# jiamiya/HOPE

Hardware: AMD Instinct MI355X
Metric: parallel env steps/sec (full CarParking step incl. obs + RS search) (higher is better)
Workload: dtype f64

## Files before the change

hope_amd/build.py:

```python
import os
import subprocess

_HERE = os.path.dirname(os.path.abspath(__file__))
_CSRC = os.path.join(_HERE, 'csrc')
_ROOT = os.path.dirname(_HERE)
SOURCES = ['hope_env.hip', 'hope_rs.hip', 'hope_bev.hip', 'hope_scenegen.cpp']
HEADERS = ['hope_math.h', 'hope_dev.h', 'hope_internal.h', 'hope_step_kernel.h', 'hope_obs_pair.h', 'hope_motion_pair.h', 'hope_scenegen_core.h', 'hope_scenegen_kernel.h', 'hope_curriculum_core.h', 'hope_curriculum_kernel.h', 'hope_maplevel_core.h', 'hope_maplevel_kernel.h', 'hope_planner_core.h', 'hope_planner_kernel.h', 'hope_chooser_core.h', 'hope_chooser_kernel.h', 'hope_obsnorm_core.h', 'hope_obsnorm_kernel.h', 'hope_evaltrack_core.h', 'hope_evaltrack_kernel.h', os.path.join(_ROOT, 'include', 'hope_env.h')]
FLAGS = ['--offload-arch=gfx950', '-O3', '-std=c++17', '-ffp-contract=off', '-fno-fast-math', '-fPIC', '-shared',
         '-Wno-unused-value', '-pthread']


def lib_path():
    return os.environ.get('HOPE_AMD_LIB') or os.path.join(_HERE, 'libhope_env.so')


def _stale(out):
    if not os.path.exists(out):
        return True
    t = os.path.getmtime(out)
    deps = [os.path.join(_CSRC, s) for s in SOURCES] + [h if os.path.isabs(h) else os.path.join(_CSRC, h) for h in HEADERS]
    return any(os.path.getmtime(d) > t for d in deps if os.path.exists(d))


def build_extension(force=False, verbose=False):
    out = lib_path()
    if not force and not _stale(out):
        return out
    hipcc = os.environ.get('HIPCC', '/opt/rocm/bin/hipcc')
    if not os.path.exists(hipcc):
        hipcc = 'hipcc'
    extra = os.environ.get('HOPE_BUILD_DEFS', '').split()
    cmd = [hipcc] + FLAGS + extra + ['-I' + os.path.join(_ROOT, 'include'), '-I' + _CSRC] + \
          [os.path.join(_CSRC, s) for s in SOURCES] + ['-o', out]
    if verbose:
        print(' '.join(cmd))
    subprocess.check_call(cmd)
    return out
```

hope_amd/csrc/hope_obs_pair.h:

```cpp
#pragma once
#include "hope_step_kernel.h"

namespace hope {

constexpr int OP_HALF = 32;
constexpr int OP_CAP = SMALL_TILE;
static_assert(OP_CAP == OP_HALF, "one lane per obstacle slot in the near-obstacle scan");
#ifndef HOPE_PAIR_NARROW
#define HOPE_PAIR_NARROW 6
#endif
static_assert(HOPE_PAIR_NARROW * 64 <= 512, "narrow edges of one pass must fit the pair queue");
constexpr int OP_EAGER = 16;
constexpr int OP_LQ = 512;
constexpr int OP_TILE_W = 8 * OP_CAP, OP_BEST_W = 128, OP_KLIST_W = OP_CAP / 2, OP_CFL_W = OP_CAP / 8;
constexpr int OP_HALF_W = OP_TILE_W + OP_BEST_W + OP_KLIST_W + OP_CFL_W;
constexpr size_t OP_LDS_BYTES = (size_t)2 * OP_HALF_W * 8 + (size_t)OP_LQ * 2;
static_assert(NACT == 42 && NBEAM == 120 && NBEAM <= 4 * OP_HALF, "lane layout of the pair kernel");

template <typename OT>
__global__ __launch_bounds__(64) void k_obs_pair(StepParams p) {
    extern __shared__ __attribute__((aligned(16))) double lds[];
    const int lane = threadIdx.x, hw = lane >> 5, hl = lane & (OP_HALF - 1);
    const int n_pairs = (p.n_list + 1) >> 1;
    if ((int)blockIdx.x >= n_pairs) return;
    const int li = 2 * scene_of_block(blockIdx.x, n_pairs) + hw;
    bool live = li < p.n_list;
    const int scene = p.scene_list[live ? li : li - 1];
    if (p.active) live = live && p.active[scene] != 0;
    if (!__any(live)) return;

    double* hbase = lds + hw * OP_HALF_W;
    double* tile = hbase;
    unsigned long long* best = (unsigned long long*)(hbase + OP_TILE_W);
    int* klist = (int*)(hbase + OP_TILE_W + OP_BEST_W);
    uint8_t* cfl = (uint8_t*)(klist + OP_CAP);
    uint16_t* queue = (uint16_t*)(lds + 2 * OP_HALF_W);

    const int n_obst = live ? min(p.n_obst[scene], OP_CAP) : 0;
    const double* st = p.state + (size_t)scene * ST_WORDS;
    const double x = st[0], y = st[1];
    const double ct = p.cs[2 * (size_t)scene], sn = p.cs[2 * (size_t)scene + 1];
    const float4* obb_s = p.obb + (size_t)scene * p.max_obst;
    float4 bb = make_float4(0.0f, 0.0f, 0.0f, 0.0f);
    if (hl < OP_EAGER) bb = obb_s[hl];
    const uint8_t gfl = (p.eflag + (size_t)scene * eflag_stride(p.max_obst))[hl];
    const double2* src = (const double2*)(p.verts + (size_t)scene * p.max_obst * 8);

    if (hl >= OP_EAGER && hl < n_obst) bb = obb_s[hl];
    const double lr = LIDAR_RANGE + 1e-6;
    const bool near = hl < n_obst && !((double)bb.x > x + lr || (double)bb.y < x - lr || (double)bb.z > y + lr || (double)bb.w < y - lr);
    int n_l;
    {
        const unsigned long long m = __ballot(near);
        const unsigned hm = hw ? (unsigned)(m >> 32) : (unsigned)m;
        n_l = __popc(hm);
        if (near) {
            const int pos = __popc(hm & ((1u << hl) - 1));
            klist[pos] = hl;
            cfl[pos] = gfl;
        }
    }
    ssync();
    for (int i = hl; i < 4 * n_l; i += OP_HALF) ((double2*)tile)[i] = src[4 * klist[i >> 2] + (i & 3)];
    double base[4], pm[4];
#pragma unroll
    for (int r = 0; r < 4; r++) {
        const int bi = hl + OP_HALF * r;
        base[r] = bi < NBEAM ? p.hull_base[bi] : 0.0;
        pm[r] = bi < NBEAM ? (HOPE_MASK_LUT ? p.mask_bsc[bi] : p.pmax[UPS * bi]) : 0.0;
    }
#pragma unroll
    for (int r = 0; r < 4; r++) best[hl + OP_HALF * r] = 0x7ff0000000000000ull;
    ssync();
    {
        const double a = ct, b = sn;
        const double x_off = -x * a - y * b;
        const double y_off = x * b - y * a;
        for (int i = hl; i < 4 * n_l; i += OP_HALF) {
            const double px = tile[2 * i], py = tile[2 * i + 1];
            tile[2 * i] = a * px + b * py + x_off;
            tile[2 * i + 1] = (-b) * px + a * py + y_off;
        }
    }
    ssync();
    const int nl_max = max(__builtin_amdgcn_readlane(n_l, 0), __builtin_amdgcn_readlane(n_l, OP_HALF));
    int n_k = 0;
    for (int base_i = 0; base_i < 4 * nl_max; base_i += OP_HALF) {
        const int i = base_i + hl;
        const bool in = i < 4 * n_l;
        const int o = in ? i >> 2 : 0;
        double dd = INFINITY;
        bool amb;
        {
            bool keep_c = false, drop_c = false;
            if (in) {
                const int e = 4 * o + (i & 3), e2 = 4 * o + ((i + 1) & 3);
                const double ax = tile[2 * e], ay = tile[2 * e + 1], bx = tile[2 * e2], by = tile[2 * e2 + 1];
                const double ddx = bx - ax, ddy = by - ay;
                const double len2 = ddx * ddx + ddy * ddy;
                const double dot = (0.0 - ax) * ddx + (0.0 - ay) * ddy;
                const double qa = ax * ax + ay * ay, qb = bx * bx + by * by;
                const double num = ay * ddx - ax * ddy;
                const double R2 = LIDAR_RANGE * LIDAR_RANGE, ETA = 1e-9;
                const double lo = R2 * (1.0 - ETA), hi = R2 * (1.0 + ETA);
                const double n2 = num * num;
                const bool line_far = n2 > hi * len2, line_near = n2 < lo * len2;
                const bool foot_in = dot > ETA * len2 && dot < (1.0 - ETA) * len2;
                const bool foot_a = dot < -ETA * len2, foot_b = dot > (1.0 + ETA) * len2;
                keep_c = qa < lo || qb < lo || (foot_in && line_near);
                drop_c = !keep_c && (len2 > 0.0 ? (line_far || (foot_a && qa > hi) || (foot_b && qb > hi)) : qa > hi);
            }
            const unsigned long long kb = __ballot(keep_c), db = __ballot(drop_c);
            const int sh = lane & ~3;
            const bool ring_keep = ((kb >> sh) & 0xF) != 0, ring_drop = ((db >> sh) & 0xF) == 0xF;
            if (ring_keep) dd = 0.0;
            amb = in && !ring_keep && !ring_drop;
        }
        if (__any(amb)) {
            if (amb) {
                const int e = 4 * o + (i & 3), e2 = 4 * o + ((i + 1) & 3);
                dd = origin_seg_dist(tile[2 * e], tile[2 * e + 1], tile[2 * e2], tile[2 * e2 + 1]);
            }
            dd = fmin(dd, dpp_d<0xB1>(dd));
            dd = fmin(dd, dpp_d<0x4E>(dd));
        }
        const bool kq = in && (i & 3) == 0 && dd < LIDAR_RANGE;
        const unsigned long long km = __ballot(kq);
        const unsigned hkm = hw ? (unsigned)(km >> 32) : (unsigned)km;
        if (kq) klist[n_k + __popc(hkm & ((1u << hl) - 1))] = o;
        n_k += __popc(hkm);
    }
    ssync();
    const int n_kslots = 4 * n_k;
    const int nk_max = max(__builtin_amdgcn_readlane(n_kslots, 0), __builtin_amdgcn_readlane(n_kslots, OP_HALF));

    int qn = 0;
    auto drain = [&]() {
        ssync();
        for (int q0 = 0; q0 < qn; q0 += WAVE) {
            const int q = q0 + lane;
            if (q < qn) {
                const int pr = queue[q];
                const int bi = pr & 127, e = (pr >> 7) & 127, hh = pr >> 14;
                const int e2 = (e & ~3) | ((e + 1) & 3);
                const double* tl = lds + hh * OP_HALF_W;
                const double x1 = tl[2 * e], y1 = tl[2 * e + 1], x2 = tl[2 * e2], y2 = tl[2 * e2 + 1];
                const double d = y2 - y1, ee = x1 - x2, f = y1 * x2 - x1 * y2;
                const double ba = p.beam_ab[2 * bi], bb_ = p.beam_ab[2 * bi + 1];
                double r = INFINITY;
                if (beam_may_hit(ba, bb_, x1, y1, x2, y2)) r = beam_edge(bi, ba, bb_, x1, y1, x2, y2, d, ee, f);
                if (r < INFINITY) atomicMin((unsigned long long*)(tl + OP_TILE_W) + bi, (unsigned long long)__double_as_longlong(r));
            }
        }
        ssync();
        qn = 0;
    };
    {
        const float PITCH = 6.283185307179586f / NBEAM, MARGIN = 2e-3f;
        for (int base_i = 0; base_i < nk_max && !(p.stages & STAGE_NO_BEAMS); base_i += OP_HALF) {
            const int i = base_i + hl;
            const bool in = i < n_kslots;
            const int e = in ? 4 * klist[i >> 2] + (i & 3) : 0;
            int lo = 0, cnt = 0;
            bool front = false, back = false, risky = true;
            if (in) {
                const int e2 = (e & ~3) | ((e + 1) & 3);
                const double dx1 = tile[2 * e], dy1 = tile[2 * e + 1], dx2 = tile[2 * e2], dy2 = tile[2 * e2 + 1];
                const float x1 = (float)dx1, y1 = (float)dy1;
                const float x2 = (float)dx2, y2 = (float)dy2;
                const float t1 = span_angle(y1, x1);
                const float t2 = __int_as_float(__builtin_amdgcn_mov_dpp(__float_as_int(t1), 0x39, 0xf, 0xf, true));
                float dth = t2 - t1;
                if (dth > 3.14159265f) dth -= 6.28318531f;
                if (dth <= -3.14159265f) dth += 6.28318531f;
                const float span = fabsf(dth);
                const bool wild = span > 3.13f || !(span == span) || fminf(x1 * x1 + y1 * y1, x2 * x2 + y2 * y2) < 0.01f;
                if (wild) { lo = 0; cnt = NBEAM; }
                else {
                    float ts = dth >= 0 ? t1 : t2;
                    if (ts < 0) ts += 6.28318531f;
                    const int ilo = (int)ceilf((ts - MARGIN) * (1.0f / PITCH));
                    const int ihi = (int)floorf((ts + span + MARGIN) * (1.0f / PITCH));
                    cnt = ihi - ilo + 1;
                    if (cnt < 0) cnt = 0;
                    if (cnt > NBEAM) cnt = NBEAM;
                    lo = ilo < 0 ? ilo + NBEAM : ilo >= NBEAM ? ilo - NBEAM : ilo;
                    if ((unsigned)lo >= (unsigned)NBEAM) { lo = 0; cnt = NBEAM; }
                }
                const int fl = (int)cfl[e >> 2];
                const double cr = dx1 * dy2 - dx2 * dy1;
                const double sc2 = (dx1 * dx1 + dy1 * dy1) * (dx2 * dx2 + dy2 * dy2);
                const bool decisive = cr * cr > 1e-12 * sc2;
                const bool left = cr > 0;
                front = decisive && (left != ((fl & OBST_F_CCW) != 0));
                back = decisive && !front;
                const float q1 = t1 * (1.0f / PITCH);
                const bool near_beam = fabsf(q1 - rintf(q1)) * PITCH <= 2.0e-4f + 1e-5f;
                const bool thin = front && (fabs(dx2 - dx1) < 1e-4 || fabs(dy2 - dy1) < 1e-4);
                risky = wild || !decisive || near_beam || thin || !(fl & OBST_F_CONVEX);
            }
            {
                const unsigned long long rb = __ballot(risky), fb = __ballot(front), bb2 = __ballot(back);
                const int sh = lane & ~3;
                const bool ring_ok = ((rb >> sh) & 0xF) == 0 && ((fb >> sh) & 0xF) != 0 && ((bb2 >> sh) & 0xF) != 0;
                if (ring_ok && back && !(p.stages & STAGE_NO_CULL)) cnt = 0;
            }
            constexpr int NARROW = HOPE_PAIR_NARROW;
            const int tag = (hw << 14) | (e << 7);
            const int cs = (cnt > 0 && cnt <= NARROW) ? cnt : 0;
            const int incl = wave_incl_scan_i(cs, lane);
            const int total = __builtin_amdgcn_readlane(incl, WAVE - 1);
            if (total > 0) {
                if (qn + total > OP_LQ) drain();
                const int off = qn + incl - cs;
#pragma unroll
                for (int k = 0; k < NARROW; k++) {
                    if (k < cs) {
                        int bi = lo + k;
                        if (bi >= NBEAM) bi -= NBEAM;
                        queue[off + k] = (uint16_t)(tag | bi);
                    }
                }
                qn += total;
            }
            unsigned long long todo = __ballot(cnt > NARROW);
            while (todo) {
                const int el = __ffsll((long long)todo) - 1;
                todo &= todo - 1;
                const int lo_e = __builtin_amdgcn_readlane(lo, el), cnt_e = __builtin_amdgcn_readlane(cnt, el);
                if (qn + cnt_e > OP_LQ) drain();
                const int tag_e = __builtin_amdgcn_readlane(tag, el);
                if (lane < cnt_e) {
                    int bi = lo_e + lane;
                    if (bi >= NBEAM) bi -= NBEAM;
                    queue[qn + lane] = (uint16_t)(tag_e | bi);
                }
                if (cnt_e > WAVE && lane + WAVE < cnt_e) {
                    int bi = lo_e + lane + WAVE;
                    if (bi >= NBEAM) bi -= NBEAM;
                    queue[qn + lane + WAVE] = (uint16_t)(tag_e | bi);
                }
                qn += cnt_e;
            }
        }
    }
    if (qn > 0) drain();
    else ssync();

    double lid[4];
#pragma unroll
    for (int r = 0; r < 4; r++) {
        const int bi = hl + OP_HALF * r;
        const double bq = sqrt(__longlong_as_double((long long)best[bi < NBEAM ? bi : 0]));
        lid[r] = clipd(bq, 0, LIDAR_RANGE) - base[r];
    }
    if (p.lidar && live) {
        OT* lo_ = (OT*)p.lidar + (size_t)NBEAM * scene;
#pragma unroll
        for (int r = 0; r < 4; r++) {
            const int bi = hl + OP_HALF * r;
            if (bi < NBEAM) lo_[bi] = (OT)lid[r];
        }
    }
    if (!p.action_mask || (p.stages & STAGE_NO_MASK)) return;

    ssync();
    double* xs = (double*)best;
    double xv_own[4];
#pragma unroll
    for (int r = 0; r < 4; r++) {
        const int bi = hl + OP_HALF * r;
        xv_own[r] = clipd(lid[r], 0, 10) + base[r];
        if (bi < NBEAM) xs[bi] = xv_own[r];
    }
    if (hl == 0) xs[NBEAM] = xv_own[0];
    constexpr int HALF_ACT = NACT / 2;
    const bool alane = hl < HALF_ACT;
    int ms[2] = {NITER, NITER};
    bool tie = false;
#if HOPE_MASK_LUT
    uint32_t* alist = (uint32_t*)tile;
    int n_act = 0;
#pragma unroll
    for (int r = 0; r < 4; r++) {
        const int bi = hl + OP_HALF * r;
        const double q = (xv_own[r] - (base[r] - 1e-6)) * pm[r];
        const bool c = live && bi < NBEAM && q < (double)MASK_LUT_NB;
        const unsigned long long m = __ballot(c);
        const unsigned hm = hw ? (unsigned)(m >> 32) : (unsigned)m;
        if (c) alist[n_act + __popc(hm & ((1u << hl) - 1))] = (uint32_t)(bi << 16) | (uint32_t)(bi * MASK_LUT_NB + (int)q);
        n_act += __popc(hm);
    }
    ssync();
    const int na_max = max(__builtin_amdgcn_readlane(n_act, 0), __builtin_amdgcn_readlane(n_act, OP_HALF));
    if (na_max > 0) {
        constexpr uint32_t NONE = (uint32_t)(NBEAM * MASK_LUT_NB);
        const char* lutb = (const char*)p.mask_lut + 2 * hl;
        unsigned mlo[2] = {NITER, NITER}, mhi[2] = {NITER, NITER};
        constexpr int PG = 8;
        unsigned pk[PG / 2];
        {
            unsigned v0[PG];
#pragma unroll
            for (int g = 0; g < PG; g++) {
                const uint32_t e = g < n_act ? alist[g] & 0xFFFFu : NONE;
                v0[g] = *(const uint16_t*)(lutb + e * (MASK_LUT_ROW * 2u));
            }
#pragma unroll
            for (int g = 0; g < PG; g++) {
                mlo[0] = min(mlo[0], v0[g] & 15u); mhi[0] = min(mhi[0], (v0[g] >> 4) & 15u);
                mlo[1] = min(mlo[1], (v0[g] >> 8) & 15u); mhi[1] = min(mhi[1], v0[g] >> 12);
            }
#pragma unroll
            for (int g = 0; g < PG / 2; g++) pk[g] = v0[2 * g] | v0[2 * g + 1] << 16;
        }
        for (int k0 = PG; k0 < na_max; k0 += PG) {
            unsigned v[PG];
#pragma unroll
            for (int g = 0; g < PG; g++) {
                const uint32_t e = k0 + g < n_act ? alist[k0 + g] & 0xFFFFu : NONE;
                v[g] = *(const uint16_t*)(lutb + e * (MASK_LUT_ROW * 2u));
            }
#pragma unroll
            for (int g = 0; g < PG; g++) {
                mlo[0] = min(mlo[0], v[g] & 15u); mhi[0] = min(mhi[0], (v[g] >> 4) & 15u);
                mlo[1] = min(mlo[1], (v[g] >> 8) & 15u); mhi[1] = min(mhi[1], v[g] >> 12);
            }
        }
        if (__any(mlo[0] < mhi[0] || mlo[1] < mhi[1])) {
// ... 181 lines not shown
```

hope_amd/csrc/hope_step_kernel.h:

```cpp
#pragma once
#include "hope_dev.h"
#ifndef HOPE_PART0_OCC
#define HOPE_PART0_OCC 4
#endif
#ifndef HOPE_KIN_PRIO
#define HOPE_KIN_PRIO 3
#endif
#ifndef HOPE_MASK_MG
#define HOPE_MASK_MG 4
#endif
#include "hope_env.h"
#include "hope_internal.h"
#ifndef HOPE_STEP_SYNC_FULL
#define HOPE_STEP_SYNC_FULL 0
#endif
#ifndef HOPE_MASK_LUT
#define HOPE_MASK_LUT 1
#endif
#ifndef HOPE_MASK_FRAC_TABLE
#define HOPE_MASK_FRAC_TABLE 0
#endif

namespace hope {

// ... 389 lines not shown
    }
    return false;
}

constexpr float SPAN_ANGLE_C[6] = {0.9999772310256958f, -0.33262282609939575f, 0.19354036450386047f,
                                   -0.11642643809318542f, 0.05264730006456375f, -0.01171911507844925f};
__device__ __forceinline__ float span_angle(float y, float x) {
    const float ax = fabsf(x), ay = fabsf(y);
    const float mx = fmaxf(ax, ay), mn = fminf(ax, ay);
    const float t = mn * __builtin_amdgcn_rcpf(mx);
    const float s = t * t;
    float q = __builtin_fmaf(s, SPAN_ANGLE_C[5], SPAN_ANGLE_C[4]);
    q = __builtin_fmaf(q, s, SPAN_ANGLE_C[3]);
    q = __builtin_fmaf(q, s, SPAN_ANGLE_C[2]);
    q = __builtin_fmaf(q, s, SPAN_ANGLE_C[1]);
    q = __builtin_fmaf(q, s, SPAN_ANGLE_C[0]);
    float r = q * t;
    if (ay > ax) r = 1.57079633f - r;
    if (x < 0.0f) r = 3.14159265f - r;
    return copysignf(r, y);
}

__device__ __forceinline__ double origin_seg_dist(double ax, double ay, double bx, double by) {
    if (ax == bx && ay == by) return sqrt(ax * ax + ay * ay);
    double len2 = (bx - ax) * (bx - ax) + (by - ay) * (by - ay);
    double r = ((0.0 - ax) * (bx - ax) + (0.0 - ay) * (by - ay)) / len2;
    if (r <= 0.0) return sqrt(ax * ax + ay * ay);
    if (r >= 1.0) return sqrt(bx * bx + by * by);
    double s = ((ay - 0.0) * (bx - ax) - (ax - 0.0) * (by - ay)) / len2;
    return fabs(s) * sqrt(len2);
}

__device__ __forceinline__ bool beam_may_hit(double a, double b, double x1, double y1, double x2, double y2) {
    double s1 = a * x1 + b * y1, s2 = a * x2 + b * y2;
    const double eps = 1e-9, back = -1e-6;
    if ((s1 > eps && s2 > eps) || (s1 < -eps && s2 < -eps)) return false;
    double t1 = a * y1 - b * x1, t2 = a * y2 - b * x2;
    if (t1 < back && t2 < back) return false;
    return true;
}

__device__ __forceinline__ double beam_edge(int i, double a, double b, double x1, double y1, double x2, double y2,
                                            double d, double e, double f) {
    double det = a * e - b * d;
    if (det == 0) return INFINITY;
    double raw_x = (b * f) / det;
    double raw_y = (-(a * f)) / det;
    const double tz = 1e-8;
    const double sx = (i < NBEAM / 4 || i >= NBEAM / 4 * 3) ? 1.0 : -1.0, sy = (i < NBEAM / 2) ? 1.0 : -1.0;
    bool ok = !(sx * raw_x < -tz) && !(sy * raw_y < -tz);
    ok = ok && !(raw_x > fmax(x1, x2)) && !(raw_x < fmin(x1, x2));
    ok = ok && !(raw_y > fmax(y1, y2)) && !(raw_y < fmin(y1, y2));
    return ok ? raw_x * raw_x + raw_y * raw_y : INFINITY;
}

constexpr int KIN_SCENES_PER_BLOCK = WAVE / 4;

__constant__ const double MASK_STEP_FRACTION[NITER + 1] = {0.0 / NITER, 1.0 / NITER, 2.0 / NITER, 3.0 / NITER, 4.0 / NITER, 5.0 / NITER,
                                                           6.0 / NITER, 7.0 / NITER, 8.0 / NITER, 9.0 / NITER, 10.0 / NITER};
static_assert(NITER == 10, "MASK_STEP_FRACTION lists NITER + 1 quotients");

__device__ __forceinline__ int wave_incl_scan_i(int x, int lane) {
    x += __builtin_amdgcn_update_dpp(0, x, 0x111, 0xf, 0xf, false);
    x += __builtin_amdgcn_update_dpp(0, x, 0x112, 0xf, 0xf, false);
    x += __builtin_amdgcn_update_dpp(0, x, 0x114, 0xf, 0xf, false);
    x += __builtin_amdgcn_update_dpp(0, x, 0x118, 0xf, 0xf, false);
    const int t0 = __builtin_amdgcn_readlane(x, 15), t1 = __builtin_amdgcn_readlane(x, 31), t2 = __builtin_amdgcn_readlane(x, 47);
    return x + (lane >= 16 ? t0 : 0) + (lane >= 32 ? t1 : 0) + (lane >= 48 ? t2 : 0);
}

template <int CTRL>
__device__ __forceinline__ double dpp_d(double v) {
    const int hi = __builtin_amdgcn_mov_dpp(__double2hiint(v), CTRL, 0xf, 0xf, true);
    const int lo = __builtin_amdgcn_mov_dpp(__double2loint(v), CTRL, 0xf, 0xf, true);
    return __hiloint2double(hi, lo);
}

template <int J>
__device__ __forceinline__ double quad_bcast(double v) {
    const int hi = __builtin_amdgcn_mov_dpp(__double2hiint(v), J * 0x55, 0xf, 0xf, true);
    const int lo = __builtin_amdgcn_mov_dpp(__double2loint(v), J * 0x55, 0xf, 0xf, true);
    return __hiloint2double(hi, lo);
}

static_assert(MINI_ITER == 20, "div_by_20");
__device__ __forceinline__ double div_by_20(double x) {
    const double R = 0.05;
    const double q0 = x * R;
    const double r = fma(-q0, 20.0, x);
    return copysign(fma(r, R, q0), x);
}

template <typename AT>
__device__ __forceinline__ void kin_controls(const void* actions, int scene, uint32_t stages, double& speed, double& dh) {
    const AT* act = (const AT*)actions;
    const double a0 = (double)act[2 * (size_t)scene], a1 = (double)act[2 * (size_t)scene + 1];
    double steer = a0;
    speed = a1;
    if (!(stages & HOPE_ACTION_PHYSICAL)) {
        if (sizeof(AT) == 4 && (stages & HOPE_ACTION_RESCALE_F32)) {
            const float f0 = fminf(fmaxf((float)a0, -1.0f), 1.0f), f1 = fminf(fmaxf((float)a1, -1.0f), 1.0f);
            steer = (double)(f0 * ((float)STEER_HI - (float)STEER_LO) / 2.0f + ((float)STEER_HI + (float)STEER_LO) / 2.0f);
            speed = (double)(f1 * ((float)SPEED_HI - (float)SPEED_LO) / 2.0f + ((float)SPEED_HI + (float)SPEED_LO) / 2.0f);
        } else {
            steer = clipd(a0, -1, 1) * (STEER_HI - STEER_LO) / 2 + (STEER_HI + STEER_LO) / 2;
            speed = clipd(a1, -1, 1) * (SPEED_HI - SPEED_LO) / 2 + (SPEED_HI + SPEED_LO) / 2;
        }
    }
    speed = clipd(speed, SPEED_LO, SPEED_HI);
    steer = clipd(steer, STEER_LO, STEER_HI);
    dh = speed * hm_tan(steer) / WHEEL_BASE * STEP_LENGTH / MINI_ITER;
}

template <typename AT>
__global__ __launch_bounds__(64) void k_kinematics(int n, const int32_t* scene_list, const double* state, const void* actions,
                                                  const uint8_t* active, uint32_t stages, const double* scene_c, double* kin) {
    if (HOPE_KIN_PRIO) __builtin_amdgcn_s_setprio(HOPE_KIN_PRIO);
    __shared__ double buf[KIN_SCENES_PER_BLOCK * KIN_WORDS];
    __shared__ double terms[MINI_ITER][2 * KIN_SCENES_PER_BLOCK];
    __shared__ int sid[KIN_SCENES_PER_BLOCK];
#ifdef HOPE_KIN_PAD
    __shared__ double kin_pad[HOPE_KIN_PAD];
    if (n < 0) kin_pad[threadIdx.x] = 0.0, kin[0] = kin_pad[(threadIdx.x * 7) % HOPE_KIN_PAD];
#endif
    const int lane = threadIdx.x, q = lane & 3, ls = lane >> 2;
    const int idx = blockIdx.x * KIN_SCENES_PER_BLOCK + ls;
    const int scene = idx < n ? (scene_list ? scene_list[idx] : idx) : -1;
    const bool live = scene >= 0 && !(active && !active[scene]);
    if (__all(!live)) return;
    if (q == 0) sid[ls] = live ? scene : -1;
    const int sc_ = live ? scene : 0;
    const double* st = state + (size_t)sc_ * ST_WORDS;
    double h = st[2];
    double acc = 0.0;
    if (lane < 2 * KIN_SCENES_PER_BLOCK) {
        const int idx2 = blockIdx.x * KIN_SCENES_PER_BLOCK + (lane >> 1);
        const int sc2 = idx2 < n ? (scene_list ? scene_list[idx2] : idx2) : 0;
        acc = state[(size_t)sc2 * ST_WORDS + (lane & 1)];
    }
    double speed, dh;
    kin_controls<AT>(actions, sc_, stages, speed, dh);
    double* out = buf + ls * KIN_WORDS;
    for (int i = 0; i < q; i++) h = h + dh;
    constexpr int KJ = MINI_ITER / 4;
    static_assert(MINI_ITER % 4 == 0, "micro-steps per lane and round");
#pragma unroll 1
    for (int r = 0; r < NUM_STEP; r++) {
        double hj[KJ], sj[KJ], cj[KJ];
        hj[0] = h;
#pragma unroll
        for (int j = 1; j < KJ; j++) { double t = hj[j - 1]; t = t + dh; t = t + dh; t = t + dh; t = t + dh; hj[j] = t; }
#pragma unroll
        for (int j = 0; j < KJ; j++) hm_sincos(hj[j], &sj[j], &cj[j]);
        if (q == 0 && r > 0) {
            const int k = r - 1;
            out[k] = hj[0]; out[10 + k] = cj[0]; out[20 + k] = sj[0];
        }
#pragma unroll
        for (int j = 0; j < KJ; j++) {
            terms[4 * j + q][2 * ls] = div_by_20(speed * cj[j] * STEP_LENGTH);
            terms[4 * j + q][2 * ls + 1] = div_by_20(speed * sj[j] * STEP_LENGTH);
        }
        ssync();
        if (lane < 2 * KIN_SCENES_PER_BLOCK) {
#pragma unroll
            for (int m = 0; m < MINI_ITER; m++) acc += terms[m][lane];
// ... 436 lines not shown
            pr[0] = prev_x; pr[1] = prev_y; pr[2] = prev_h; pr[3] = fin_x; pr[4] = fin_y; pr[5] = fin_h; pr[6] = fin_ua;
            const int fl = ((p.stages & HOPE_STAGE_REWARD) ? POST_F_REWARD : 0) | (turnover ? POST_F_TURNOVER : 0) | (need_ua ? POST_F_NEED_UA : 0);
            pr[7] = __hiloint2double(fl, status | (fin_t << 8));
        }
    }

    }
    if (PART == 1 || !(p.stages & HOPE_STAGE_OBS)) { ST_T(2); ST_FLUSH(); return; }

    ST_T(2);
    int* llist = keep;
    ssync();
    const double lr = LIDAR_RANGE + 1e-6;
    const uint8_t* eflag_s = p.eflag + (size_t)scene * eflag_stride(p.max_obst);
    const int n_l = PART == 2 ? stage_near(obb_s, src, n_obst, x - lr, x + lr, y - lr, y + lr, tile, llist, lane, eflag_s, cfl, &obb_pre)
                              : build_near_list(tile, n_obst, x, y, lr, llist, lane);
    ssync();
    {
        const double a = ct, b = sn;
        const double x_off = -x * a - y * b;
        const double y_off = x * b - y * a;
        for (int i = lane; i < 4 * n_l; i += WAVE) {
            const int v = 4 * llist[i >> 2] + (i & 3);
            double px = tile[2 * v], py = tile[2 * v + 1];
            tile[2 * v] = a * px + b * py + x_off;
            tile[2 * v + 1] = (-b) * px + a * py + y_off;
        }
    }
    ssync();
    int n_k = 0;
    for (int base = 0; base < 4 * n_l; base += WAVE) {
        const int i = base + lane;
        const bool in = i < 4 * n_l;
        const int o = in ? llist[i >> 2] : 0;
        double dd = INFINITY;
        bool amb = in;
        if (!TIMING) {
            bool keep_c = false, drop_c = false;
            if (in) {
                const int e = 4 * o + (i & 3), e2 = 4 * o + ((i + 1) & 3);
                const double ax = tile[2 * e], ay = tile[2 * e + 1], bx = tile[2 * e2], by = tile[2 * e2 + 1];
                const double ddx = bx - ax, ddy = by - ay;
                const double len2 = ddx * ddx + ddy * ddy;
                const double dot = (0.0 - ax) * ddx + (0.0 - ay) * ddy;
                const double qa = ax * ax + ay * ay, qb = bx * bx + by * by;
                const double num = ay * ddx - ax * ddy;
                const double R2 = LIDAR_RANGE * LIDAR_RANGE, ETA = 1e-9;
                const double lo = R2 * (1.0 - ETA), hi = R2 * (1.0 + ETA);
                const double n2 = num * num;
                const bool line_far = n2 > hi * len2, line_near = n2 < lo * len2;
                const bool foot_in = dot > ETA * len2 && dot < (1.0 - ETA) * len2;
                const bool foot_a = dot < -ETA * len2, foot_b = dot > (1.0 + ETA) * len2;
                keep_c = qa < lo || qb < lo || (foot_in && line_near);
                drop_c = !keep_c && (len2 > 0.0 ? (line_far || (foot_a && qa > hi) || (foot_b && qb > hi)) : qa > hi);
            }
            const unsigned long long kb = __ballot(keep_c), db = __ballot(drop_c);
            const int sh = lane & ~3;
            const bool ring_keep = ((kb >> sh) & 0xF) != 0, ring_drop = ((db >> sh) & 0xF) == 0xF;
            if (ring_keep) dd = 0.0;
            amb = in && !ring_keep && !ring_drop;
        }
        if (__any(amb)) {
            if (amb) {
                const int e = 4 * o + (i & 3), e2 = 4 * o + ((i + 1) & 3);
                dd = origin_seg_dist(tile[2 * e], tile[2 * e + 1], tile[2 * e2], tile[2 * e2 + 1]);
            }
            dd = fmin(dd, dpp_d<0xB1>(dd));
            dd = fmin(dd, dpp_d<0x4E>(dd));
        }
        if (TIMING && in && (i & 3) == 0) { cen_ring_n += 1; cen_ring = fmin(cen_ring, fabs(dd - LIDAR_RANGE)); }
        const bool kq = in && (i & 3) == 0 && dd < LIDAR_RANGE;
        const unsigned long long km = __ballot(kq);
        if (kq) llist[n_k + __popcll(km & ((1ull << lane) - 1))] = o;
        n_k += __popcll(km);
    }
    ssync();
    const int n_kslots = 4 * n_k;
    ST_T(3);
    const int i0 = lane, i1 = lane + 64;
    const bool has1 = i1 < NBEAM;
    const double a0 = PART == 2 ? bm0 : p.beam_ab[2 * i0], b0 = PART == 2 ? bm1 : p.beam_ab[2 * i0 + 1];
    const double a1 = PART == 2 ? bm2 : (has1 ? p.beam_ab[2 * i1] : 0.0), b1 = PART == 2 ? bm3 : (has1 ? p.beam_ab[2 * i1 + 1] : 0.0);
    unsigned long long* best = (unsigned long long*)(scr + LDS_TX);
    int* queue = (int*)(scr + LDS_TX + 128);
    constexpr int LQ = 384;
    best[lane] = 0x7ff0000000000000ull;
    best[lane + 64] = 0x7ff0000000000000ull;
    ssync();
    int qn = 0;
    auto drain = [&]() {
        const unsigned long long td_ = TIMING ? __builtin_readcyclecounter() : 0;
        ssync();
        for (int q0 = 0; q0 < qn; q0 += WAVE) {
            int q = q0 + lane;
            if (q < qn) {
                int pr = queue[q];
                int bi = pr & 127, e = pr >> 7;
                int e2 = (e & ~3) | ((e + 1) & 3);
                double x1 = tile[2 * e], y1 = tile[2 * e + 1], x2 = tile[2 * e2], y2 = tile[2 * e2 + 1];
                double d = y2 - y1, ee = x1 - x2, f = y1 * x2 - x1 * y2;
                const double ba = p.beam_ab[2 * bi], bb = p.beam_ab[2 * bi + 1];
                double r = INFINITY;
                if (beam_may_hit(ba, bb, x1, y1, x2, y2)) r = beam_edge(bi, ba, bb, x1, y1, x2, y2, d, ee, f);
                if (r < INFINITY) atomicMin(&best[bi], (unsigned long long)__double_as_longlong(r));
            }
        }
        ssync();
        qn = 0;
        if (TIMING) { const unsigned long long dt_ = __builtin_readcyclecounter() - td_; tsec[6] += dt_; t0_ += dt_; }
    };
    {
        const float PITCH = 6.283185307179586f / NBEAM, MARGIN = 2e-3f;
        for (int base = 0; base < n_kslots && !(p.stages & STAGE_NO_BEAMS); base += WAVE) {
            const int i = base + lane;
            const int e = i < n_kslots ? 4 * llist[i >> 2] + (i & 3) : 0;
            int lo = 0, cnt = 0;
            bool front = false, back = false, risky = true;
            if (i < n_kslots) {
                const int e2 = (e & ~3) | ((e + 1) & 3);
                const double dx1 = tile[2 * e], dy1 = tile[2 * e + 1], dx2 = tile[2 * e2], dy2 = tile[2 * e2 + 1];
                const float x1 = (float)dx1, y1 = (float)dy1;
                const float x2 = (float)dx2, y2 = (float)dy2;
                const float t1 = span_angle(y1, x1);
                const float t2 = __int_as_float(__builtin_amdgcn_mov_dpp(__float_as_int(t1), 0x39, 0xf, 0xf, true));
                float dth = t2 - t1;
                if (dth > 3.14159265f) dth -= 6.28318531f;
                if (dth <= -3.14159265f) dth += 6.28318531f;
                const float span = fabsf(dth);
                const bool wild = span > 3.13f || !(span == span) || fminf(x1 * x1 + y1 * y1, x2 * x2 + y2 * y2) < 0.01f;
                if (wild) { lo = 0; cnt = NBEAM; }
                else {
                    float ts = dth >= 0 ? t1 : t2;
                    if (ts < 0) ts += 6.28318531f;
                    const int ilo = (int)ceilf((ts - MARGIN) * (1.0f / PITCH));
                    const int ihi = (int)floorf((ts + span + MARGIN) * (1.0f / PITCH));
                    cnt = ihi - ilo + 1;
                    if (cnt < 0) cnt = 0;
                    if (cnt > NBEAM) cnt = NBEAM;
                    lo = ilo < 0 ? ilo + NBEAM : ilo >= NBEAM ? ilo - NBEAM : ilo;
                    if ((unsigned)lo >= (unsigned)NBEAM) { lo = 0; cnt = NBEAM; }
                }
                const int fl = (int)cfl[e >> 2];
                const double cr = dx1 * dy2 - dx2 * dy1;
                const double sc2 = (dx1 * dx1 + dy1 * dy1) * (dx2 * dx2 + dy2 * dy2);
                const bool decisive = cr * cr > 1e-12 * sc2;
                const bool left = cr > 0;
                front = decisive && (left != ((fl & OBST_F_CCW) != 0));
                back = decisive && !front;
                const float q1 = t1 * (1.0f / PITCH);
                const bool near_beam = fabsf(q1 - rintf(q1)) * PITCH <= 2.0e-4f + 1e-5f;
                const bool thin = front && (fabs(dx2 - dx1) < 1e-4 || fabs(dy2 - dy1) < 1e-4);
                risky = wild || !decisive || near_beam || thin || !(fl & OBST_F_CONVEX);
            }
            {
                const unsigned long long rb = __ballot(risky), fb = __ballot(front), bb = __ballot(back);
                const int sh = lane & ~3;
                const bool ring_ok = ((rb >> sh) & 0xF) == 0 && ((fb >> sh) & 0xF) != 0 && ((bb >> sh) & 0xF) != 0;
                if (ring_ok && back && !(p.stages & STAGE_NO_CULL)) cnt = 0;
            }
            ST_T(4);
            constexpr int NARROW = 6;
            const int cs = (cnt > 0 && cnt <= NARROW) ? cnt : 0;
            const int incl = wave_incl_scan_i(cs, lane);
            const int total = __builtin_amdgcn_readlane(incl, WAVE - 1);
            if (total > 0) {
                if (qn + total > LQ) drain();
                const int off = qn + incl - cs, tag = e << 7;
#pragma unroll
                for (int k = 0; k < NARROW; k++) {
                    if (k < cs) {
                        int bi = lo + k;
                        if (bi >= NBEAM) bi -= NBEAM;
                        queue[off + k] = tag | bi;
                    }
                }
                qn += total;
            }
            unsigned long long todo = __ballot(cnt > NARROW);
            while (todo) {
                const int el = __ffsll((long long)todo) - 1;
                todo &= todo - 1;
                const int lo_e = __builtin_amdgcn_readlane(lo, el), cnt_e = __builtin_amdgcn_readlane(cnt, el);
                if (qn + cnt_e > LQ) drain();
                const int tag = __builtin_amdgcn_readlane(e, el) << 7;
                if (lane < cnt_e) {
                    int bi = lo_e + lane;
                    if (bi >= NBEAM) bi -= NBEAM;
                    queue[qn + lane] = tag | bi;
                }
                if (cnt_e > WAVE && lane + WAVE < cnt_e) {
                    int bi = lo_e + lane + WAVE;
                    if (bi >= NBEAM) bi -= NBEAM;
                    queue[qn + lane + WAVE] = tag | bi;
                }
                qn += cnt_e;
            }
            ST_T(5);
        }
    }
    constexpr bool MLUT = HOPE_MASK_LUT && !TIMING;
    const double pm0 = MLUT ? p.mask_bsc[i0] : p.pmax[UPS * i0], pm1 = has1 ? (MLUT ? p.mask_bsc[i1] : p.pmax[UPS * i1]) : 0.0;
    if (qn > 0) drain();
    const double best0 = sqrt(__longlong_as_double((long long)best[i0]));
    const double best1 = has1 ? sqrt(__longlong_as_double((long long)best[i1])) : INFINITY;
    const double base0 = p.hull_base[i0], base1 = has1 ? p.hull_base[i1] : 0.0;
    const double lid0 = clipd(best0, 0, LIDAR_RANGE) - base0;
    const double lid1 = clipd(best1, 0, LIDAR_RANGE) - base1;
    if (p.lidar) {
        OT* lo = (OT*)p.lidar + (size_t)NBEAM * scene;
        lo[i0] = (OT)lid0;
        if (has1) lo[i1] = (OT)lid1;
    }
    ST_T(5);
    if (!p.action_mask || (p.stages & STAGE_NO_MASK)) { ST_FLUSH(); return; }

    ssync();
    double* xs = scr + LDS_X;
    xs[i0] = clipd(lid0, 0, 10) + base0;
    if (has1) xs[i1] = clipd(lid1, 0, 10) + base1;
    ssync();
    if (lane == 0) xs[NBEAM] = xs[0];
    ssync();
    int mstep = NITER;
    bool tie = false, mask_trivial = false;
    if (MLUT) {
        const double q0 = (xs[i0] - (base0 - 1e-6)) * pm0, q1 = has1 ? (xs[i1] - (base1 - 1e-6)) * pm1 : (double)MASK_LUT_NB;
        const bool c0 = q0 < (double)MASK_LUT_NB, c1 = has1 && q1 < (double)MASK_LUT_NB;
        const int row0 = i0 * MASK_LUT_NB + (c0 ? (int)q0 : 0), row1 = i1 * MASK_LUT_NB + (c1 ? (int)q1 : 0);
        const unsigned long long am[2] = {__ballot(c0), __ballot(c1)};
        mask_trivial = !(am[0] | am[1]);
        if (am[0] | am[1]) {
            constexpr int NONE = NBEAM * MASK_LUT_NB;
            const int hl_ = lane < NACT / 2 ? lane : (lane < NACT ? lane - NACT / 2 : 31), sh_ = (lane >= NACT / 2 && lane < NACT) ? 8 : 0;
            const char* lutb = (const char*)p.mask_lut + 2 * hl_;
            unsigned mlo = NITER, mhi = NITER;
            constexpr int PG = 8;
            unsigned long long m0 = am[0], m1 = am[1];
            auto pop_row = [&]() -> int {
                int row = NONE;
                if (m0) { const int l_ = __ffsll((long long)m0) - 1; m0 &= m0 - 1; row = __builtin_amdgcn_readlane(row0, l_); }
                else if (m1) { const int l_ = __ffsll((long long)m1) - 1; m1 &= m1 - 1; row = __builtin_amdgcn_readlane(row1, l_); }
                return row;
            };
            unsigned pk[PG / 2];
            {
                unsigned v0[PG];
#pragma unroll
                for (int g = 0; g < PG; g++) v0[g] = (unsigned)*(const uint16_t*)(lutb + (unsigned)pop_row() * (MASK_LUT_ROW * 2u)) >> sh_ & 0xFFu;
#pragma unroll
                for (int g = 0; g < PG; g++) { mlo = min(mlo, v0[g] & 15u); mhi = min(mhi, v0[g] >> 4); }
#pragma unroll
                for (int g = 0; g < PG / 2; g++) pk[g] = v0[2 * g] | v0[2 * g + 1] << 16;
            }
            while (m0 | m1) {
                unsigned v[PG];
#pragma unroll
                for (int g = 0; g < PG; g++) v[g] = (unsigned)*(const uint16_t*)(lutb + (unsigned)pop_row() * (MASK_LUT_ROW * 2u)) >> sh_ & 0xFFu;
#pragma unroll
                for (int g = 0; g < PG; g++) { mlo = min(mlo, v[g] & 15u); mhi = min(mhi, v[g] >> 4); }
            }
            if (__any(mlo < mhi)) {
                const char* tabb = (const char*)p.tab;
                int k = 0;
#pragma unroll
                for (int half = 0; half < 2; half++) {
                    unsigned long long m = am[half];
                    while (m) {
                        const int l_ = __ffsll((long long)m) - 1;
                        m &= m - 1;
                        const int ib = 64 * half + l_;
                        unsigned w;
                        switch (k >> 1) {
                            case 0: w = pk[0]; break; case 1: w = pk[1]; break; case 2: w = pk[2]; break; case 3: w = pk[3]; break;
                            default: {
                                const int row = __builtin_amdgcn_readlane(half ? row1 : row0, l_);
                                w = ((unsigned)*(const uint16_t*)(lutb + (unsigned)row * (MASK_LUT_ROW * 2u)) >> sh_ & 0xFFu) << ((k & 1) << 4);
                            }
                        }
                        w = (w >> ((k & 1) << 4)) & 0xFFu;
                        k++;
                        const unsigned lo = w & 15u, hi = w >> 4;
                        const bool need = lo < hi && lo < mhi;
                        if (!__any(need)) continue;
                        const double xv = xs[ib];
                        if (need) {
// ... 247 lines not shown
```

Baseline: 158.5 million.

## Replace per-pair lidar queue with run-length queue and skip hit prefilter for non-wild edges

Replaces the per-(edge,beam) pair queue in the lidar stage with a run-length queue. Each edge now appends one packed run descriptor plus a start mark, instead of one queue entry per beam. Drain expands runs with a wave max-scan over the marks. The two-path narrow/wide enqueue with serialized per-edge readlane loops is removed, and the beam_may_hit prefilter is skipped for non-wild edges whose beam range is already tight. This cuts enqueue work and LDS writes, at the cost of a DPP scan per drain chunk, and relies on the angular range being exact enough to drop the prefilter.

```diff
diff --git a/hope_amd/build.py b/hope_amd/build.py
--- a/hope_amd/build.py
+++ b/hope_amd/build.py
@@ -5,7 +5,7 @@
 _CSRC = os.path.join(_HERE, 'csrc')
 _ROOT = os.path.dirname(_HERE)
 SOURCES = ['hope_env.hip', 'hope_rs.hip', 'hope_bev.hip', 'hope_scenegen.cpp']
-HEADERS = ['hope_math.h', 'hope_dev.h', 'hope_internal.h', 'hope_step_kernel.h', 'hope_obs_pair.h', 'hope_motion_pair.h', 'hope_scenegen_core.h', 'hope_scenegen_kernel.h', 'hope_curriculum_core.h', 'hope_curriculum_kernel.h', 'hope_maplevel_core.h', 'hope_maplevel_kernel.h', 'hope_planner_core.h', 'hope_planner_kernel.h', 'hope_chooser_core.h', 'hope_chooser_kernel.h', 'hope_obsnorm_core.h', 'hope_obsnorm_kernel.h', 'hope_evaltrack_core.h', 'hope_evaltrack_kernel.h', os.path.join(_ROOT, 'include', 'hope_env.h')]
+HEADERS = ['hope_math.h', 'hope_dev.h', 'hope_internal.h', 'hope_step_kernel.h', 'hope_lidar_runs_core.h', 'hope_lidar_runs.h', 'hope_obs_pair.h', 'hope_motion_pair.h', 'hope_scenegen_core.h', 'hope_scenegen_kernel.h', 'hope_curriculum_core.h', 'hope_curriculum_kernel.h', 'hope_maplevel_core.h', 'hope_maplevel_kernel.h', 'hope_planner_core.h', 'hope_planner_kernel.h', 'hope_chooser_core.h', 'hope_chooser_kernel.h', 'hope_obsnorm_core.h', 'hope_obsnorm_kernel.h', 'hope_evaltrack_core.h', 'hope_evaltrack_kernel.h', os.path.join(_ROOT, 'include', 'hope_env.h')]
 FLAGS = ['--offload-arch=gfx950', '-O3', '-std=c++17', '-ffp-contract=off', '-fno-fast-math', '-fPIC', '-shared',
          '-Wno-unused-value', '-pthread']
 
diff --git a/hope_amd/csrc/hope_lidar_runs.h b/hope_amd/csrc/hope_lidar_runs.h
--- /dev/null
+++ b/hope_amd/csrc/hope_lidar_runs.h
@@ -0,0 +1,93 @@
+#pragma once
+#include "hope_lidar_runs_core.h"
+
+namespace hope {
+
+static_assert(LR_NBEAM == NBEAM && LR_WAVE == WAVE, "hope_lidar_runs_core.h restates the beam count and the wave size");
+constexpr size_t LR_LDS_BYTES = (size_t)LR_RUNS * 4 + LR_CAP;
+
+struct LidarRuns {
+    uint32_t* info;
+    uint8_t* mark;
+    int qslots, nruns;
+};
+
+__device__ __forceinline__ void lr_init(LidarRuns& Q, void* mem, int lane) {
+    Q.info = (uint32_t*)mem;
+    Q.mark = (uint8_t*)(Q.info + LR_RUNS);
+    Q.qslots = 0;
+    Q.nruns = 0;
+    static_assert(LR_CAP / 4 == 2 * WAVE, "two words of marks per lane");
+    ((uint32_t*)Q.mark)[lane] = 0;
+    ((uint32_t*)Q.mark)[lane + WAVE] = 0;
+}
+
+__device__ __forceinline__ int wave_incl_max_i(int x) {
+    x = lr_join(x, __builtin_amdgcn_update_dpp(0, x, 0x111, 0xf, 0xf, false));
+    x = lr_join(x, __builtin_amdgcn_update_dpp(0, x, 0x112, 0xf, 0xf, false));
+    x = lr_join(x, __builtin_amdgcn_update_dpp(0, x, 0x114, 0xf, 0xf, false));
+    x = lr_join(x, __builtin_amdgcn_update_dpp(0, x, 0x118, 0xf, 0xf, false));
+    x = lr_join(x, __builtin_amdgcn_update_dpp(0, x, 0x142, 0xa, 0xf, false));
+    x = lr_join(x, __builtin_amdgcn_update_dpp(0, x, 0x143, 0xc, 0xf, false));
+    return x;
+}
+
+template <class PairFn>
+__device__ __forceinline__ void lr_drain(LidarRuns& Q, int lane, PairFn pair) {
+    ssync();
+    int carry = 0;
+    for (int q0 = 0; q0 < Q.qslots; q0 += WAVE) {
+        const int q = q0 + lane;
+        int m = Q.mark[q];
+        Q.mark[q] = 0;
+        m = lr_join(wave_incl_max_i(m), carry);
+        carry = __builtin_amdgcn_readlane(m, WAVE - 1);
+        if (q < Q.qslots) {
+            const uint32_t in = Q.info[m - 1];
+            pair(in, lr_beam(in, q));
+        }
+    }
+    ssync();
+    Q.qslots = 0;
+    Q.nruns = 0;
+}
+
+template <class DrainFn>
+__device__ __forceinline__ void lr_append(LidarRuns& Q, int lane, int half, int e, int lo, int cnt, bool wild, DrainFn drain) {
+    const int incl = wave_incl_scan_i(cnt, lane);
+    const bool has = cnt > 0;
+    const unsigned long long hm = __ballot(has);
+    if (hm == 0) return;
+    const int rank = __popcll(hm & ((1ull << lane) - 1));
+    unsigned long long pend = hm;
+    int done_s = 0, done_r = 0;
+    while (pend) {
+        const bool fit = ((pend >> lane) & 1) && lr_fits(Q.qslots + (incl - done_s), Q.nruns + (rank - done_r));
+        const unsigned long long fm = __ballot(fit);
+        if (fm == 0) { drain(); continue; }
+        if (fit) {
+            const int run = Q.nruns + rank - done_r, first = Q.qslots + incl - cnt - done_s;
+            Q.info[run] = lr_pack(half, e, lo, first, wild);
+            Q.mark[first] = (uint8_t)(run + 1);
+        }
+        const int end_s = __builtin_amdgcn_readlane(incl, 63 - __clzll((long long)fm));
+        const int n = __popcll(fm);
+        Q.qslots += end_s - done_s;
+        done_s = end_s;
+        Q.nruns += n;
+        done_r += n;
+        pend &= ~fm;
+    }
+}
+
+__device__ __forceinline__ void lidar_pair(const double* tile, unsigned long long* best, const double* beam_ab, int e, int bi, bool wild) {
+    const int e2 = (e & ~3) | ((e + 1) & 3);
+    const double x1 = tile[2 * e], y1 = tile[2 * e + 1], x2 = tile[2 * e2], y2 = tile[2 * e2 + 1];
+    const double d = y2 - y1, ee = x1 - x2, f = y1 * x2 - x1 * y2;
+    const double ba = beam_ab[2 * bi], bb = beam_ab[2 * bi + 1];
+    double r = INFINITY;
+    if (!wild || beam_may_hit(ba, bb, x1, y1, x2, y2)) r = beam_edge(bi, ba, bb, x1, y1, x2, y2, d, ee, f);
+    if (r < INFINITY) atomicMin(best + bi, (unsigned long long)__double_as_longlong(r));
+}
+
+}
diff --git a/hope_amd/csrc/hope_lidar_runs_core.h b/hope_amd/csrc/hope_lidar_runs_core.h
--- /dev/null
+++ b/hope_amd/csrc/hope_lidar_runs_core.h
@@ -0,0 +1,100 @@
+#pragma once
+#include <stdint.h>
+
+#if defined(__HIPCC__) || defined(__CUDACC__)
+#define LR_HD __host__ __device__ inline
+#else
+#define LR_HD inline
+#endif
+
+constexpr int LR_NBEAM = 120;
+constexpr int LR_WAVE = 64;
+constexpr int LR_CAP = 512;
+constexpr int LR_RUNS = 128;
+static_assert(LR_CAP % LR_WAVE == 0 && LR_NBEAM <= LR_CAP && LR_RUNS < 256 && LR_CAP <= 512, "run queue layout");
+
+LR_HD uint32_t lr_pack(int half, int edge, int lo, int first, bool wild) {
+    return (uint32_t)first | (uint32_t)lo << 9 | (uint32_t)edge << 16 | (uint32_t)half << 26 | (uint32_t)(wild ? 1 : 0) << 27;
+}
+LR_HD int lr_first(uint32_t info) { return (int)(info & 511u); }
+LR_HD int lr_lo(uint32_t info) { return (int)((info >> 9) & 127u); }
+LR_HD int lr_edge(uint32_t info) { return (int)((info >> 16) & 1023u); }
+LR_HD int lr_half(uint32_t info) { return (int)((info >> 26) & 1u); }
+LR_HD bool lr_wild(uint32_t info) { return ((info >> 27) & 1u) != 0; }
+
+LR_HD int lr_beam(uint32_t info, int slot) {
+    const int b = lr_lo(info) + (slot - lr_first(info));
+    return b >= LR_NBEAM ? b - LR_NBEAM : b;
+}
+
+LR_HD bool lr_fits(int slots_after, int run) { return slots_after <= LR_CAP && run < LR_RUNS; }
+
+LR_HD int lr_join(int a, int b) { return a > b ? a : b; }
+
+#if !defined(__HIP_DEVICE_COMPILE__)
+struct LrHostQueue {
+    uint8_t mark[LR_CAP];
+    uint32_t info[LR_RUNS];
+    int qslots, nruns;
+    long drains;
+};
+inline void lr_host_init(LrHostQueue* q) {
+    for (int i = 0; i < LR_CAP; i++) q->mark[i] = 0;
+    q->qslots = q->nruns = 0;
+    q->drains = 0;
+}
+template <class Emit>
+inline void lr_host_drain(LrHostQueue* q, Emit emit) {
+    int carry = 0;
+    for (int q0 = 0; q0 < q->qslots; q0 += LR_WAVE) {
+        int m[LR_WAVE];
+        for (int lane = 0; lane < LR_WAVE; lane++) {
+            m[lane] = q->mark[q0 + lane];
+            q->mark[q0 + lane] = 0;
+        }
+        for (int lane = 1; lane < LR_WAVE; lane++) m[lane] = lr_join(m[lane], m[lane - 1]);
+        for (int lane = 0; lane < LR_WAVE; lane++) m[lane] = lr_join(m[lane], carry);
+        carry = m[LR_WAVE - 1];
+        for (int lane = 0; lane < LR_WAVE; lane++) {
+            const int s = q0 + lane;
+            if (s >= q->qslots) continue;
+            const uint32_t in = q->info[m[lane] - 1];
+            emit(lr_half(in), lr_edge(in), lr_beam(in, s), lr_wild(in));
+        }
+    }
+    q->qslots = q->nruns = 0;
+    q->drains++;
+}
+template <class Emit>
+inline void lr_host_append(LrHostQueue* q, int n, const int* half, const int* edge, const int* lo, const int* cnt, const int* wild, Emit emit) {
+    int incl[LR_WAVE], rank[LR_WAVE];
+    bool pend[LR_WAVE];
+    int s = 0, r = 0, n_pend = 0;
+    for (int k = 0; k < n; k++) {
+        rank[k] = r;
+        s += cnt[k];
+        incl[k] = s;
+        pend[k] = cnt[k] > 0;
+        if (pend[k]) { r++; n_pend++; }
+    }
+    int done_s = 0, done_r = 0;
+    while (n_pend > 0) {
+        int n_fit = 0, last = -1;
+        for (int k = 0; k < n; k++) {
+            if (!pend[k] || !lr_fits(q->qslots + (incl[k] - done_s), q->nruns + (rank[k] - done_r))) continue;
+            const int run = q->nruns + rank[k] - done_r, first = q->qslots + incl[k] - cnt[k] - done_s;
+            q->info[run] = lr_pack(half[k], edge[k], lo[k], first, wild[k] != 0);
+            q->mark[first] = (uint8_t)(run + 1);
+            pend[k] = false;
+            n_fit++;
+            last = k;
+        }
+        if (n_fit == 0) { lr_host_drain(q, emit); continue; }
+        q->qslots += incl[last] - done_s;
+        done_s = incl[last];
+        q->nruns += n_fit;
+        done_r += n_fit;
+        n_pend -= n_fit;
+    }
+}
+#endif
diff --git a/hope_amd/csrc/hope_obs_pair.h b/hope_amd/csrc/hope_obs_pair.h
--- a/hope_amd/csrc/hope_obs_pair.h
+++ b/hope_amd/csrc/hope_obs_pair.h
@@ -6,15 +6,10 @@
 constexpr int OP_HALF = 32;
 constexpr int OP_CAP = SMALL_TILE;
 static_assert(OP_CAP == OP_HALF, "one lane per obstacle slot in the near-obstacle scan");
-#ifndef HOPE_PAIR_NARROW
-#define HOPE_PAIR_NARROW 6
-#endif
-static_assert(HOPE_PAIR_NARROW * 64 <= 512, "narrow edges of one pass must fit the pair queue");
 constexpr int OP_EAGER = 16;
-constexpr int OP_LQ = 512;
 constexpr int OP_TILE_W = 8 * OP_CAP, OP_BEST_W = 128, OP_KLIST_W = OP_CAP / 2, OP_CFL_W = OP_CAP / 8;
 constexpr int OP_HALF_W = OP_TILE_W + OP_BEST_W + OP_KLIST_W + OP_CFL_W;
-constexpr size_t OP_LDS_BYTES = (size_t)2 * OP_HALF_W * 8 + (size_t)OP_LQ * 2;
+constexpr size_t OP_LDS_BYTES = (size_t)2 * OP_HALF_W * 8 + LR_LDS_BYTES;
 static_assert(NACT == 42 && NBEAM == 120 && NBEAM <= 4 * OP_HALF, "lane layout of the pair kernel");
 
 template <typename OT>
@@ -134,26 +129,13 @@
     const int n_kslots = 4 * n_k;
     const int nk_max = max(__builtin_amdgcn_readlane(n_kslots, 0), __builtin_amdgcn_readlane(n_kslots, OP_HALF));
 
-    int qn = 0;
+    LidarRuns rq;
+    lr_init(rq, lds + 2 * OP_HALF_W, lane);
     auto drain = [&]() {
-        ssync();
-        for (int q0 = 0; q0 < qn; q0 += WAVE) {
-            const int q = q0 + lane;
-            if (q < qn) {
-                const int pr = queue[q];
-                const int bi = pr & 127, e = (pr >> 7) & 127, hh = pr >> 14;
-                const int e2 = (e & ~3) | ((e + 1) & 3);
-                const double* tl = lds + hh * OP_HALF_W;
-                const double x1 = tl[2 * e], y1 = tl[2 * e + 1], x2 = tl[2 * e2], y2 = tl[2 * e2 + 1];
-                const double d = y2 - y1, ee = x1 - x2, f = y1 * x2 - x1 * y2;
-                const double ba = p.beam_ab[2 * bi], bb_ = p.beam_ab[2 * bi + 1];
-                double r = INFINITY;
-                if (beam_may_hit(ba, bb_, x1, y1, x2, y2)) r = beam_edge(bi, ba, bb_, x1, y1, x2, y2, d, ee, f);
-                if (r < INFINITY) atomicMin((unsigned long long*)(tl + OP_TILE_W) + bi, (unsigned long long)__double_as_longlong(r));
-            }
-        }
-        ssync();
-        qn = 0;
+        lr_drain(rq, lane, [&](uint32_t in, int bi) {
+            const double* tl = lds + lr_half(in) * OP_HALF_W;
+            lidar_pair(tl, (unsigned long long*)(tl + OP_TILE_W), p.beam_ab, lr_edge(in), bi, lr_wild(in));
+        });
     };
     {
         const float PITCH = 6.283185307179586f / NBEAM, MARGIN = 2e-3f;
@@ -162,7 +144,7 @@
             const bool in = i < n_kslots;
             const int e = in ? 4 * klist[i >> 2] + (i & 3) : 0;
             int lo = 0, cnt = 0;
-            bool front = false, back = false, risky = true;
+            bool front = false, back = false, risky = true, wild_e = false;
             if (in) {
                 const int e2 = (e & ~3) | ((e + 1) & 3);
                 const double dx1 = tile[2 * e], dy1 = tile[2 * e + 1], dx2 = tile[2 * e2], dy2 = tile[2 * e2 + 1];
@@ -175,6 +157,7 @@
                 if (dth <= -3.14159265f) dth += 6.28318531f;
                 const float span = fabsf(dth);
                 const bool wild = span > 3.13f || !(span == span) || fminf(x1 * x1 + y1 * y1, x2 * x2 + y2 * y2) < 0.01f;
+                wild_e = wild;
                 if (wild) { lo = 0; cnt = NBEAM; }
                 else {
                     float ts = dth >= 0 ? t1 : t2;
@@ -205,46 +188,10 @@
                 const bool ring_ok = ((rb >> sh) & 0xF) == 0 && ((fb >> sh) & 0xF) != 0 && ((bb2 >> sh) & 0xF) != 0;
                 if (ring_ok && back && !(p.stages & STAGE_NO_CULL)) cnt = 0;
             }
-            constexpr int NARROW = HOPE_PAIR_NARROW;
-            const int tag = (hw << 14) | (e << 7);
-            const int cs = (cnt > 0 && cnt <= NARROW) ? cnt : 0;
-            const int incl = wave_incl_scan_i(cs, lane);
-            const int total = __builtin_amdgcn_readlane(incl, WAVE - 1);
-            if (total > 0) {
-                if (qn + total > OP_LQ) drain();
-                const int off = qn + incl - cs;
-#pragma unroll
-                for (int k = 0; k < NARROW; k++) {
-                    if (k < cs) {
-                        int bi = lo + k;
-                        if (bi >= NBEAM) bi -= NBEAM;
-                        queue[off + k] = (uint16_t)(tag | bi);
-                    }
-                }
-                qn += total;
-            }
-            unsigned long long todo = __ballot(cnt > NARROW);
-            while (todo) {
-                const int el = __ffsll((long long)todo) - 1;
-                todo &= todo - 1;
-                const int lo_e = __builtin_amdgcn_readlane(lo, el), cnt_e = __builtin_amdgcn_readlane(cnt, el);
-                if (qn + cnt_e > OP_LQ) drain();
-                const int tag_e = __builtin_amdgcn_readlane(tag, el);
-                if (lane < cnt_e) {
-                    int bi = lo_e + lane;
-                    if (bi >= NBEAM) bi -= NBEAM;
-                    queue[qn + lane] = (uint16_t)(tag_e | bi);
-                }
-                if (cnt_e > WAVE && lane + WAVE < cnt_e) {
-                    int bi = lo_e + lane + WAVE;
-                    if (bi >= NBEAM) bi -= NBEAM;
-                    queue[qn + lane + WAVE] = (uint16_t)(tag_e | bi);
-                }
-                qn += cnt_e;
-            }
-        }
-    }
-    if (qn > 0) drain();
+            lr_append(rq, lane, hw, e, lo, cnt, wild_e, drain);
+        }
+    }
+    if (rq.qslots > 0) drain();
     else ssync();
 
     double lid[4];
diff --git a/hope_amd/csrc/hope_step_kernel.h b/hope_amd/csrc/hope_step_kernel.h
--- a/hope_amd/csrc/hope_step_kernel.h
+++ b/hope_amd/csrc/hope_step_kernel.h
@@ -495,6 +495,10 @@
     const int lo = __builtin_amdgcn_mov_dpp(__double2loint(v), J * 0x55, 0xf, 0xf, true);
     return __hiloint2double(hi, lo);
 }
+
+}
+#include "hope_lidar_runs.h"
+namespace hope {
 
 static_assert(MINI_ITER == 20, "div_by_20");
 __device__ __forceinline__ double div_by_20(double x) {
@@ -1097,31 +1101,15 @@
     const double a0 = PART == 2 ? bm0 : p.beam_ab[2 * i0], b0 = PART == 2 ? bm1 : p.beam_ab[2 * i0 + 1];
     const double a1 = PART == 2 ? bm2 : (has1 ? p.beam_ab[2 * i1] : 0.0), b1 = PART == 2 ? bm3 : (has1 ? p.beam_ab[2 * i1 + 1] : 0.0);
     unsigned long long* best = (unsigned long long*)(scr + LDS_TX);
-    int* queue = (int*)(scr + LDS_TX + 128);
-    constexpr int LQ = 384;
+    static_assert(128 * 8 + LR_LDS_BYTES <= 320 * 8, "best[] and the run queue share region A");
+    LidarRuns rq;
+    lr_init(rq, scr + LDS_TX + 128, lane);
     best[lane] = 0x7ff0000000000000ull;
     best[lane + 64] = 0x7ff0000000000000ull;
     ssync();
-    int qn = 0;
     auto drain = [&]() {
         const unsigned long long td_ = TIMING ? __builtin_readcyclecounter() : 0;
-        ssync();
-        for (int q0 = 0; q0 < qn; q0 += WAVE) {
-            int q = q0 + lane;
-            if (q < qn) {
-                int pr = queue[q];
-                int bi = pr & 127, e = pr >> 7;
-                int e2 = (e & ~3) | ((e + 1) & 3);
-                double x1 = tile[2 * e], y1 = tile[2 * e + 1], x2 = tile[2 * e2], y2 = tile[2 * e2 + 1];
-                double d = y2 - y1, ee = x1 - x2, f = y1 * x2 - x1 * y2;
-                const double ba = p.beam_ab[2 * bi], bb = p.beam_ab[2 * bi + 1];
-                double r = INFINITY;
-                if (beam_may_hit(ba, bb, x1, y1, x2, y2)) r = beam_edge(bi, ba, bb, x1, y1, x2, y2, d, ee, f);
-                if (r < INFINITY) atomicMin(&best[bi], (unsigned long long)__double_as_longlong(r));
-            }
-        }
-        ssync();
-        qn = 0;
+        lr_drain(rq, lane, [&](uint32_t in, int bi) { lidar_pair(tile, best, p.beam_ab, lr_edge(in), bi, lr_wild(in)); });
         if (TIMING) { const unsigned long long dt_ = __builtin_readcyclecounter() - td_; tsec[6] += dt_; t0_ += dt_; }
     };
     {
@@ -1131,6 +1119,7 @@
             const int e = i < n_kslots ? 4 * llist[i >> 2] + (i & 3) : 0;
             int lo = 0, cnt = 0;
             bool front = false, back = false, risky = true;
+            bool wild_e = false;
             if (i < n_kslots) {
                 const int e2 = (e & ~3) | ((e + 1) & 3);
                 const double dx1 = tile[2 * e], dy1 = tile[2 * e + 1], dx2 = tile[2 * e2], dy2 = tile[2 * e2 + 1];
@@ -1143,6 +1132,7 @@
                 if (dth <= -3.14159265f) dth += 6.28318531f;
                 const float span = fabsf(dth);
                 const bool wild = span > 3.13f || !(span == span) || fminf(x1 * x1 + y1 * y1, x2 * x2 + y2 * y2) < 0.01f;
+                wild_e = wild;
                 if (wild) { lo = 0; cnt = NBEAM; }
                 else {
                     float ts = dth >= 0 ? t1 : t2;
@@ -1174,48 +1164,13 @@
                 if (ring_ok && back && !(p.stages & STAGE_NO_CULL)) cnt = 0;
             }
             ST_T(4);
-            constexpr int NARROW = 6;
-            const int cs = (cnt > 0 && cnt <= NARROW) ? cnt : 0;
-            const int incl = wave_incl_scan_i(cs, lane);
-            const int total = __builtin_amdgcn_readlane(incl, WAVE - 1);
-            if (total > 0) {
-                if (qn + total > LQ) drain();
-                const int off = qn + incl - cs, tag = e << 7;
-#pragma unroll
-                for (int k = 0; k < NARROW; k++) {
-                    if (k < cs) {
-                        int bi = lo + k;
-                        if (bi >= NBEAM) bi -= NBEAM;
-                        queue[off + k] = tag | bi;
-                    }
-                }
-                qn += total;
-            }
-            unsigned long long todo = __ballot(cnt > NARROW);
-            while (todo) {
-                const int el = __ffsll((long long)todo) - 1;
-                todo &= todo - 1;
-                const int lo_e = __builtin_amdgcn_readlane(lo, el), cnt_e = __builtin_amdgcn_readlane(cnt, el);
-                if (qn + cnt_e > LQ) drain();
-                const int tag = __builtin_amdgcn_readlane(e, el) << 7;
-                if (lane < cnt_e) {
-                    int bi = lo_e + lane;
-                    if (bi >= NBEAM) bi -= NBEAM;
-                    queue[qn + lane] = tag | bi;
-                }
-                if (cnt_e > WAVE && lane + WAVE < cnt_e) {
-                    int bi = lo_e + lane + WAVE;
-                    if (bi >= NBEAM) bi -= NBEAM;
-                    queue[qn + lane + WAVE] = tag | bi;
-                }
-                qn += cnt_e;
-            }
+            lr_append(rq, lane, 0, e, lo, cnt, wild_e, drain);
             ST_T(5);
         }
     }
     constexpr bool MLUT = HOPE_MASK_LUT && !TIMING;
     const double pm0 = MLUT ? p.mask_bsc[i0] : p.pmax[UPS * i0], pm1 = has1 ? (MLUT ? p.mask_bsc[i1] : p.pmax[UPS * i1]) : 0.0;
-    if (qn > 0) drain();
+    if (rq.qslots > 0) drain();
     const double best0 = sqrt(__longlong_as_double((long long)best[i0]));
     const double best1 = has1 ? sqrt(__longlong_as_double((long long)best[i1])) : INFINITY;
     const double base0 = p.hull_base[i0], base1 = has1 ? p.hull_base[i1] : 0.0;
```

Result: faster. 164.7 million, median of 6 (+3.9%).
